# shaneson0/attacking_federate_learning

Measured on AMD Instinct MI355X. Metric: aggregation rounds/sec at N clients x D params (Bulyan), higher is better.
Workload: dtype f32 (Gram: fp16x2 split of every fp32 operand, 3 fp16 MFMAs per block, fp32/fp64 accumulate; <= 2e-7 of |gi||gj| vs f...

## Files before the change

### attacking_federate_learning_amd/csrc/gram_planes.hip

```cpp
#include "common.hpp"

#include <cstring>
#include <type_traits>

namespace byz {
namespace {

constexpr int kWgRows = 256;
constexpr int kWgCols = 128;
constexpr int kSlab = 128;
constexpr int kThreads = 512;
constexpr int kFragBytes = 1024;
constexpr int kRowBlocks = (kWgRows + kWgCols) / 32;
constexpr int kChunkCols = 8192;
constexpr int kChunkSteps = kChunkCols / 16;
constexpr int kFlushSteps = 16;
constexpr int kSpareRoundsPercent = 10;

typedef float f32x16 __attribute__((ext_vector_type(16)));
typedef float f32x4 __attribute__((ext_vector_type(4)));
typedef __bf16 bf16x8 __attribute__((ext_vector_type(8)));
typedef _Float16 f16x8 __attribute__((ext_vector_type(8)));
typedef uint32_t u32x4 __attribute__((ext_vector_type(4)));

__device__ __forceinline__ void split_bf16x3(const f32x4& lo4, const f32x4& hi4, u32x4& hp, u32x4& mp, u32x4& lp) {
    uint32_t xb[8], r1b[8], r2b[8];
#pragma unroll
    for (int e = 0; e < 8; ++e) {
        const float x = e < 4 ? lo4[e] : hi4[e - 4];
        xb[e] = __float_as_uint(x);
        const float r1 = x - __uint_as_float(xb[e] & 0xffff0000u);
        r1b[e] = __float_as_uint(r1);
        const float r2 = r1 - __uint_as_float(r1b[e] & 0xffff0000u);
        r2b[e] = __float_as_uint(r2);
    }
#pragma unroll
    for (int e = 0; e < 4; ++e) {
        hp[e] = __builtin_amdgcn_perm(xb[2 * e + 1], xb[2 * e], 0x07060302u);
        mp[e] = __builtin_amdgcn_perm(r1b[2 * e + 1], r1b[2 * e], 0x07060302u);
        lp[e] = __builtin_amdgcn_perm(r2b[2 * e + 1], r2b[2 * e], 0x07060302u);
    }
}

__device__ __forceinline__ void split_f16x2(const f32x4& lo4, const f32x4& hi4, float scale, u32x4& hp, u32x4& mp) {
    f16x8 h, m;
#pragma unroll
    for (int e = 0; e < 8; ++e) {
        const float x = (e < 4 ? lo4[e] : hi4[e - 4]) * scale;
        h[e] = static_cast<_Float16>(x);
        m[e] = static_cast<_Float16>(x - static_cast<float>(h[e]));
    }
    hp = __builtin_bit_cast(u32x4, h);
    mp = __builtin_bit_cast(u32x4, m);
}

__device__ __forceinline__ f32x4 load4_tail(const float* __restrict__ src, int64_t k, int64_t n_cols) {
    f32x4 v = {0.0f, 0.0f, 0.0f, 0.0f};
    if (k + 3 < n_cols) {
        v = *reinterpret_cast<const f32x4*>(src + k);
    } else {
        if (k + 0 < n_cols) v.x = src[k + 0];
        if (k + 1 < n_cols) v.y = src[k + 1];
        if (k + 2 < n_cols) v.z = src[k + 2];
    }
    return v;
}

constexpr int kSplitCols = 128;
__global__ __launch_bounds__(256) void plane_split_bf16_kernel(const float* __restrict__ G, int64_t n_rows, int64_t n_cols,
                                                               int64_t ld, const int32_t* __restrict__ row_index,
                                                               int64_t k0, int64_t n_steps, u32x4* __restrict__ planes) {
    __shared__ __attribute__((aligned(16))) float tile[32][kSplitCols + 4];
    const int tid = threadIdx.x;
    const int64_t rb = blockIdx.y;
    const int64_t step0 = static_cast<int64_t>(blockIdx.x) * (kSplitCols / 16);
    {
        const int r = tid >> 3, c = tid & 7;
        int64_t row = rb * 32 + r;
        if (row > n_rows - 1) row = n_rows - 1;
        if (row_index != nullptr) row = row_index[row];
        const float* src = G + row * ld;
#pragma unroll
        for (int p = 0; p < 4; ++p) {
            const int col = 4 * c + 32 * p;
            *reinterpret_cast<f32x4*>(&tile[r][col]) = load4_tail(src, k0 + step0 * 16 + col, n_cols);
        }
    }
    __syncthreads();
    const int lane = tid & 63, wave = tid >> 6;
#pragma unroll
    for (int i = 0; i < 2; ++i) {
        const int sl = 2 * wave + i;
        const int64_t step = step0 + sl;
        if (step >= n_steps) continue;
        const int row = lane & 31, kk = sl * 16 + 8 * (lane >> 5);
        const f32x4 lo4 = *reinterpret_cast<const f32x4*>(&tile[row][kk]);
        const f32x4 hi4 = *reinterpret_cast<const f32x4*>(&tile[row][kk + 4]);
        u32x4 h, m, l;
        split_bf16x3(lo4, hi4, h, m, l);
        u32x4* out = planes + ((rb * n_steps + step) * 3) * 64 + lane;
        out[0] = h;
        out[64] = m;
        out[128] = l;
    }
}

__global__ __launch_bounds__(256) void plane_split_f16_kernel(const float* __restrict__ G, int64_t n_rows, int64_t n_cols,
                                                              int64_t ld, const int32_t* __restrict__ row_index, int64_t k0,
                                                              int64_t n_steps, u32x4* __restrict__ planes,
                                                              double* __restrict__ unscale, int64_t rows_pad,
                                                              const int32_t* __restrict__ redo) {
    __shared__ __attribute__((aligned(16))) float tile[32][kSplitCols + 4];
    __shared__ float row_scale[32];
    const int tid = threadIdx.x;
    const int lane = tid & 63, wave = tid >> 6;
    const int listed = redo != nullptr ? redo[0] : 1;
    for (int item = redo != nullptr ? static_cast<int>(blockIdx.x) : 0; item < listed; item += static_cast<int>(gridDim.x)) {
    const int64_t rb = redo != nullptr ? redo[2 + 2 * item] : blockIdx.y;
    const int64_t chunk = redo != nullptr ? redo[1 + 2 * item] : blockIdx.x;
    const int r = tid >> 3, c = tid & 7;
    int64_t row = rb * 32 + r;
    if (row > n_rows - 1) row = n_rows - 1;
    if (row_index != nullptr) row = row_index[row];
    const float* src = G + row * ld;
    const int64_t kbeg = k0 + chunk * kChunkCols;
    {
        float mx = 0.0f;
        bool bad = false;
#pragma unroll 8
        for (int i = 0; i < kChunkCols / 32; ++i) {
            const f32x4 v = load4_tail(src, kbeg + 4 * c + 32 * i, n_cols);
#pragma unroll
            for (int e = 0; e < 4; ++e) {
                const float a = __builtin_fabsf(v[e]);
                bad = bad || !(a <= 3.0e38f);
                mx = __builtin_fmaxf(mx, a);
            }
        }
#pragma unroll
        for (int msk = 1; msk < 8; msk <<= 1) {
            mx = __builtin_fmaxf(mx, __shfl_xor(mx, msk, 64));
            bad = bad || (__shfl_xor(bad ? 1 : 0, msk, 64) != 0);
        }
        int shift = 0;
        if (!bad && mx > 0.0f) {
            shift = 14 - (static_cast<int>((__float_as_uint(mx) >> 23) & 0xffu) - 127);
            if (mx < 1.17549435e-38f) shift = 126;
            if (shift > 126) shift = 126;
            if (shift < -126) shift = -126;
        }
        if (c == 0) {
            row_scale[r] = __uint_as_float(static_cast<uint32_t>(shift + 127) << 23);
            unscale[chunk * rows_pad + rb * 32 + r] = __longlong_as_double(static_cast<long long>(1023 - shift) << 52);
        }
    }
    __syncthreads();
    const int64_t step_base = chunk * kChunkSteps;
    for (int sub = 0; sub < kChunkCols / kSplitCols; ++sub) {
        const int64_t step0 = step_base + sub * (kSplitCols / 16);
        if (step0 >= n_steps) break;
#pragma unroll
        for (int p = 0; p < 4; ++p) {
            const int col = 4 * c + 32 * p;
            *reinterpret_cast<f32x4*>(&tile[r][col]) = load4_tail(src, k0 + step0 * 16 + col, n_cols);
        }
        __syncthreads();
#pragma unroll
        for (int i = 0; i < 2; ++i) {
            const int sl = 2 * wave + i;
            const int64_t step = step0 + sl;
            if (step >= n_steps) continue;
            const int frow = lane & 31, kk = sl * 16 + 8 * (lane >> 5);
            const f32x4 lo4 = *reinterpret_cast<const f32x4*>(&tile[frow][kk]);
            const f32x4 hi4 = *reinterpret_cast<const f32x4*>(&tile[frow][kk + 4]);
            u32x4 h, m;
            split_f16x2(lo4, hi4, row_scale[frow], h, m);
            u32x4* out = planes + ((rb * n_steps + step) * 2) * 64 + lane;
            out[0] = h;
            out[64] = m;
        }
        __syncthreads();
    }
    if (redo == nullptr) break;
    __syncthreads();
    }
}

constexpr int kSampleGroups = 16;
__global__ __launch_bounds__(256) void plane_split_f16_stream_kernel(const float* __restrict__ G, int64_t n_rows, int64_t n_cols,
                                                                     int64_t ld, const int32_t* __restrict__ row_index, int64_t k0,
                                                                     int64_t n_steps, u32x4* __restrict__ planes,
                                                                     double* __restrict__ unscale, int64_t rows_pad,
                                                                     int32_t* __restrict__ redo) {
    __shared__ __attribute__((aligned(16))) float tile[2][32][kSplitCols + 4];
    __shared__ float row_scale[32];
    __shared__ int block_bad;
    const int tid = threadIdx.x;
    const int lane = tid & 63, wave = tid >> 6;
    const int64_t rb = blockIdx.y;
    const int64_t chunk = blockIdx.x;
    const int r = tid >> 3, c = tid & 7;
    int64_t row = rb * 32 + r;
    if (row > n_rows - 1) row = n_rows - 1;
    if (row_index != nullptr) row = row_index[row];
    const float* src = G + row * ld;
    const int64_t kbeg = k0 + chunk * kChunkCols;
    if (tid == 0) block_bad = 0;
    int shift = 0;
    {
        float mx = 0.0f;
#pragma unroll
        for (int g = 0; g < 2; ++g) {
            const int64_t k = kbeg + (2 * c + g) * (kChunkCols / kSampleGroups);
            const f32x4 a = load4_tail(src, k, n_cols), b = load4_tail(src, k + 4, n_cols);
#pragma unroll
            for (int e = 0; e < 4; ++e) mx = __builtin_fmaxf(mx, __builtin_fmaxf(__builtin_fabsf(a[e]), __builtin_fabsf(b[e])));
        }
#pragma unroll
        for (int msk = 1; msk < 8; msk <<= 1) mx = __builtin_fmaxf(mx, __shfl_xor(mx, msk, 64));
        if (mx >= 1.17549435e-38f && mx <= 3.0e38f) {
            shift = 9 - (static_cast<int>((__float_as_uint(mx) >> 23) & 0xffu) - 127);
            if (shift > 126) shift = 126;
            if (shift < -126) shift = -126;
        }
        if (c == 0) row_scale[r] = __uint_as_float(static_cast<uint32_t>(shift + 127) << 23);
    }
    const int64_t step_base = chunk * kChunkSteps;
    const float scale = __uint_as_float(static_cast<uint32_t>(shift + 127) << 23);
    float true_max = 0.0f;
    bool bad = false;
    f32x4 cur[4], nxt[4];
#pragma unroll
    for (int p = 0; p < 4; ++p) cur[p] = load4_tail(src, k0 + step_base * 16 + 4 * c + 32 * p, n_cols);
    __syncthreads();
    for (int sub = 0; sub < kChunkCols / kSplitCols; ++sub) {
        const int64_t step0 = step_base + sub * (kSplitCols / 16);
        if (step0 >= n_steps) break;
        const bool more = sub + 1 < kChunkCols / kSplitCols && step0 + kSplitCols / 16 < n_steps;
        if (more) {
#pragma unroll
            for (int p = 0; p < 4; ++p) nxt[p] = load4_tail(src, k0 + (step0 + kSplitCols / 16) * 16 + 4 * c + 32 * p, n_cols);
        }
        float (*t)[kSplitCols + 4] = tile[sub & 1];
#pragma unroll
        for (int p = 0; p < 4; ++p) {
            *reinterpret_cast<f32x4*>(&t[r][4 * c + 32 * p]) = cur[p];
#pragma unroll
            for (int e = 0; e < 4; ++e) {
                const float a = __builtin_fabsf(cur[p][e]);
                bad = bad || !(a <= 3.0e38f);
                true_max = __builtin_fmaxf(true_max, a);
            }
        }
        __syncthreads();
#pragma unroll
        for (int i = 0; i < 2; ++i) {
            const int sl = 2 * wave + i;
            const int64_t step = step0 + sl;
            if (step >= n_steps) continue;
            const int frow = lane & 31, kk = sl * 16 + 8 * (lane >> 5);
            const f32x4 lo4 = *reinterpret_cast<const f32x4*>(&t[frow][kk]);
            const f32x4 hi4 = *reinterpret_cast<const f32x4*>(&t[frow][kk + 4]);
            u32x4 h, m;
            split_f16x2(lo4, hi4, row_scale[frow], h, m);
            u32x4* out = planes + ((rb * n_steps + step) * 2) * 64 + lane;
            out[0] = h;
            out[64] = m;
        }
        if (more) {
#pragma unroll
            for (int p = 0; p < 4; ++p) cur[p] = nxt[p];
        }
    }
#pragma unroll
    for (int msk = 1; msk < 8; msk <<= 1) {
        true_max = __builtin_fmaxf(true_max, __shfl_xor(true_max, msk, 64));
        bad = bad || (__shfl_xor(bad ? 1 : 0, msk, 64) != 0);
    }
    const float scaled = true_max * scale;
    const bool holds = !bad && (true_max == 0.0f || (scaled >= 128.0f && scaled < 65536.0f));
    if (c == 0) {
        unscale[chunk * rows_pad + rb * 32 + r] = __longlong_as_double(static_cast<long long>(1023 - shift) << 52);
        if (!holds) block_bad = 1;
    }
    __syncthreads();
    if (tid == 0 && block_bad != 0) {
        const int at = atomicAdd(redo, 1);
        redo[1 + 2 * at] = static_cast<int32_t>(chunk);
        redo[2 + 2 * at] = static_cast<int32_t>(rb);
    }
}

template <int N>
__device__ __forceinline__ void wait_vmcnt() {
    asm volatile("s_waitcnt vmcnt(%0)" ::"n"(N) : "memory");
}
__device__ __forceinline__ void wait_vmcnt_dyn(int n) {
    switch (n) {
#define BYZ_W(k) case k: wait_vmcnt<k>(); break;
        BYZ_W(0) BYZ_W(3) BYZ_W(4) BYZ_W(5) BYZ_W(6) BYZ_W(8) BYZ_W(9) BYZ_W(10) BYZ_W(12) BYZ_W(15) BYZ_W(16) BYZ_W(18) BYZ_W(20) BYZ_W(24)
#undef BYZ_W
        default: wait_vmcnt<0>(); break;
    }
}

struct Frags {
    bf16x8 a[3][2], b[3][2];
};

template <int NBUF>
__global__ __launch_bounds__(512, 1) void gram_planes_kernel(const u32x4* __restrict__ planes, int64_t n_steps,
                                                             double* __restrict__ partial, int n_tiles,
                                                             const int2* __restrict__ tile_order, int n_chunks,
                                                             int* __restrict__ tickets, int round_size, int t128,
                                                             int slab_live0, int n_blocks32,
                                                             int32_t* __restrict__ device_status) {
    constexpr int PLANES = 3;
    constexpr int kRbBytes = PLANES * kFragBytes;
    constexpr int kStage = kRowBlocks * kRbBytes;
    constexpr int NW = 8;
    constexpr int kPieces = kRowBlocks * PLANES;
    constexpr int kPerWave = (kPieces + NW - 1) / NW;
    constexpr int kFullWaves = kPieces % NW == 0 ? NW : kPieces % NW;
    constexpr int kLead = NBUF;
    typedef bf16x8 frag_t;
    extern __shared__ __attribute__((aligned(16))) unsigned char lds[];

    const int xcd = blockIdx.x & 7;
    const int seq = blockIdx.x >> 3;
    const int base = n_tiles >> 3, rem = n_tiles & 7;
    const int mine = base + (xcd < rem ? 1 : 0);
    const int first = xcd * base + (xcd < rem ? xcd : rem);
    const int chunk = mine > 0 ? seq / mine : n_chunks;
    int* done = tickets + n_tiles + xcd;
    {
        const int round = round_size > 0 ? seq / round_size : 0;
        if (round > 0 && threadIdx.x == 0) {
            unsigned spins = 0;
            while (__hip_atomic_load(done, __ATOMIC_RELAXED, __HIP_MEMORY_SCOPE_AGENT) < round * round_size) {
                __builtin_amdgcn_s_sleep(16);
                if (++spins > (1u << 20)) break;
            }
        }
        __syncthreads();
        if (chunk >= n_chunks) {
            if (threadIdx.x == 0) __hip_atomic_fetch_add(done, 1, __ATOMIC_RELAXED, __HIP_MEMORY_SCOPE_AGENT);
            return;
        }
    }
    const int t_list = first + (seq - chunk * mine);
    const int2 tt = tile_order[t_list];
    const int bi = __builtin_amdgcn_readfirstlane(tt.x);
    const int tj = __builtin_amdgcn_readfirstlane(tt.y);

    const int tid = threadIdx.x;
    const int lane = tid & 63;
    const int wave = __builtin_amdgcn_readfirstlane(tid >> 6);
    const int wr = wave >> 1, wc = wave & 1;
    const int ti = 2 * bi + wr / 2;
    const int row_in_slab = (wr % 2) * 64;
    unsigned live_blocks = 0;
    if (tj <= ti && ti < t128 && n_blocks32 < 0) {
        live_blocks = 15u;
    } else if (tj <= ti && ti < t128) {
#pragma unroll
        for (int m = 0; m < 2; ++m)
#pragma unroll
            for (int n = 0; n < 2; ++n) {
                const int rblk = ti * 4 + row_in_slab / 32 + m, cblk = tj * 4 + wc * 2 + n;
                if (rblk < n_blocks32 && cblk <= rblk) live_blocks |= 1u << (m * 2 + n);
            }
    }
    const bool live_wave = live_blocks != 0;

    const int step0 = chunk * kChunkSteps;
    int n_stages = static_cast<int>(n_steps) - step0;
    if (n_stages > kChunkSteps) n_stages = kChunkSteps;

    int64_t piece_off[kPerWave];
#pragma unroll
    for (int i = 0; i < kPerWave; ++i) {
        int q = wave + NW * i;
        if (q >= kPieces) q = kPieces - 1;
        const int rbl = q / PLANES, piece = q % PLANES;
        const int64_t rb = rbl < 8 ? static_cast<int64_t>(bi) * 8 + rbl : static_cast<int64_t>(tj) * 4 + (rbl - 8);
        piece_off[i] = (((rb * n_steps + step0) * PLANES + piece) * 64) * 16;
    }
    const unsigned char* lane_base = reinterpret_cast<const unsigned char*>(planes) + lane * 16;
    const int my_dmas = wave < kFullWaves ? kPerWave : kPerWave - 1;
    auto dma = [&](int s) __attribute__((always_inline)) {
        unsigned char* dst = lds + (s % NBUF) * kStage + wave * kFragBytes;
#pragma unroll
        for (int i = 0; i < kPerWave; ++i) {
            if (kFullWaves != NW && i == kPerWave - 1 && wave >= kFullWaves) break;
            __builtin_amdgcn_global_load_lds(
                (const __attribute__((address_space(1))) void*)(lane_base + piece_off[i] + static_cast<int64_t>(s) * (PLANES * kFragBytes)),
                (__attribute__((address_space(3))) void*)(dst + i * NW * kFragBytes), 16, 0, 0);
        }
    };

    f32x16 acc[2][2], acc2[2][2];
#pragma unroll
    for (int m = 0; m < 2; ++m)
#pragma unroll
        for (int n = 0; n < 2; ++n)
#pragma unroll
            for (int e = 0; e < 16; ++e) {
                acc[m][n][e] = 0.0f;
                acc2[m][n][e] = 0.0f;
            }

    auto read_frags = [&](int s, Frags& f, auto mask_c) __attribute__((always_inline)) {
        constexpr unsigned MASK = decltype(mask_c)::value;
        const unsigned char* A = lds + (s % NBUF) * kStage + (2 * wr) * kRbBytes + lane * 16;
        const unsigned char* B = lds + (s % NBUF) * kStage + (8 + 2 * wc) * kRbBytes + lane * 16;
#pragma unroll
        for (int p = 0; p < PLANES; ++p) {
#pragma unroll
            for (int m = 0; m < 2; ++m)
                if (((MASK >> (m * 2)) & 3u) != 0) f.a[p][m] = *reinterpret_cast<const frag_t*>(A + m * kRbBytes + p * kFragBytes);
#pragma unroll
            for (int n = 0; n < 2; ++n)
                if (((MASK >> n) & 5u) != 0) f.b[p][n] = *reinterpret_cast<const frag_t*>(B + n * kRbBytes + p * kFragBytes);
        }
    };
    auto multiply = [&](const Frags& f, auto mask_c) __attribute__((always_inline)) {
        constexpr unsigned MASK = decltype(mask_c)::value;
        constexpr int pa[6] = {2, 0, 1, 1, 0, 0};
        constexpr int pb[6] = {0, 2, 1, 0, 1, 0};
#pragma unroll
        for (int t = 0; t < 6; ++t)
#pragma unroll
            for (int m = 0; m < 2; ++m)
#pragma unroll
                for (int n = 0; n < 2; ++n)
                    if (((MASK >> (m * 2 + n)) & 1u) != 0)
                        acc[m][n] = __builtin_amdgcn_mfma_f32_32x32x16_bf16(f.a[pa[t]][m], f.b[pb[t]][n], acc[m][n], 0, 0, 0);
    };
    auto flush = [&](int s) __attribute__((always_inline)) {
        if ((s + 1) % kFlushSteps == 0) {
#pragma unroll
            for (int m = 0; m < 2; ++m)
#pragma unroll
                for (int n = 0; n < 2; ++n)
#pragma unroll
                    for (int e = 0; e < 16; ++e) {
                        acc2[m][n][e] += acc[m][n][e];
                        acc[m][n][e] = 0.0f;
                    }
        }
    };
    auto steady = [&](int s, const Frags& cur, Frags& next, auto mask_c) __attribute__((always_inline)) {
        constexpr bool kLive = decltype(mask_c)::value != 0;
        dma(s + kLead);
        if (kLive) {
            read_frags(s + 1, next, mask_c);
            multiply(cur, mask_c);
        }
        if (kFullWaves == NW || wave < kFullWaves) wait_vmcnt<(kLead - 2) * kPerWave>();
        else wait_vmcnt<(kLead - 2) * (kPerWave - 1)>();
        asm volatile("s_waitcnt lgkmcnt(0)\n\ts_barrier" ::: "memory");
        if (kLive) flush(s);
    };
    auto drain = [&](int s, const Frags& cur, Frags& next, auto mask_c) __attribute__((always_inline)) {
        constexpr bool kLive = decltype(mask_c)::value != 0;
        if (s + kLead < n_stages) dma(s + kLead);
        if (kLive) {
            if (s + 1 < n_stages) read_frags(s + 1, next, mask_c);
            multiply(cur, mask_c);
        }
        const int last = s + kLead < n_stages ? s + kLead : n_stages - 1;
        const int ahead = last - (s + 2);
        wait_vmcnt_dyn((ahead > 0 ? ahead : 0) * my_dmas);
        asm volatile("s_waitcnt lgkmcnt(0)\n\ts_barrier" ::: "memory");
        if (kLive) flush(s);
    };

    for (int a = 0; a < kLead && a < n_stages; ++a) dma(a);
    {
        const int issued = n_stages < kLead ? n_stages : kLead;
        wait_vmcnt_dyn((issued > 2 ? issued - 2 : 0) * my_dmas);
    }
    asm volatile("s_barrier" ::: "memory");
    auto k_loop = [&](auto mask_c) __attribute__((always_inline)) {
        constexpr bool kLive = decltype(mask_c)::value != 0;
        Frags x, y;
        if (kLive && n_stages > 0) read_frags(0, x, mask_c);
        asm volatile("s_waitcnt lgkmcnt(0)\n\ts_barrier" ::: "memory");
        int s = 0;
        for (; s + 1 + kLead < n_stages; s += 2) {
            steady(s, x, y, mask_c);
            steady(s + 1, y, x, mask_c);
        }
        for (; s < n_stages; s += 2) {
            drain(s, x, y, mask_c);
            if (s + 1 < n_stages) drain(s + 1, y, x, mask_c);
        }
    };
    switch (live_blocks) {
        case 0u: k_loop(std::integral_constant<unsigned, 0u>{}); break;
        case 1u: k_loop(std::integral_constant<unsigned, 1u>{}); break;
        case 3u: k_loop(std::integral_constant<unsigned, 3u>{}); break;
        case 13u: k_loop(std::integral_constant<unsigned, 13u>{}); break;
        default: live_blocks = 15u; k_loop(std::integral_constant<unsigned, 15u>{}); break;
    }
    auto block_live = [&](int m, int n) __attribute__((always_inline)) { return ((live_blocks >> (m * 2 + n)) & 1u) != 0; };

    bool lost = false;
    if (chunk > 0) {
        if (tid == 0) {
            unsigned spins = 0;
            while (__hip_atomic_load(tickets + t_list, __ATOMIC_RELAXED, __HIP_MEMORY_SCOPE_AGENT) != chunk) {
                __builtin_amdgcn_s_sleep(8);
                if (++spins > (1u << 26)) {
                    lost = true;
                    break;
                }
            }
            __builtin_amdgcn_fence(__ATOMIC_ACQUIRE, "agent");
        }
        lost = __syncthreads_or(lost ? 1 : 0) != 0;
    }
    if (lost) {
        if (tid == 0) atomicOr(device_status, kStatusLostTicket);
    } else if (live_wave) {
        const bool slab_live = chunk > 0 || slab_live0 != 0;
        double* out = partial + (static_cast<int64_t>(ti) * (ti + 1) / 2 + tj) * (kSlab * kSlab);
#pragma unroll
        for (int m = 0; m < 2; ++m)
#pragma unroll
            for (int n = 0; n < 2; ++n) {
                if (!block_live(m, n)) continue;
                const int j = wc * 64 + n * 32 + (lane & 31);
#pragma unroll
                for (int e = 0; e < 16; ++e) {
                    const int i = row_in_slab + m * 32 + (e & 3) + 8 * (e >> 2) + 4 * (lane >> 5);
                    double v = static_cast<double>(acc2[m][n][e]);
                    v += static_cast<double>(acc[m][n][e]);
                    if (slab_live) v += out[i * kSlab + j];
                    out[i * kSlab + j] = v;
                }
            }
    }
    asm volatile("s_waitcnt vmcnt(0)" ::: "memory");
    __syncthreads();
    if (tid == 0) {
        __builtin_amdgcn_fence(__ATOMIC_RELEASE, "agent");
        asm volatile("s_waitcnt vmcnt(0)" ::: "memory");
        __hip_atomic_store(tickets + t_list, chunk + 1, __ATOMIC_RELAXED, __HIP_MEMORY_SCOPE_AGENT);
        __hip_atomic_fetch_add(done, 1, __ATOMIC_RELAXED, __HIP_MEMORY_SCOPE_AGENT);
    }
}

template <int NBUF, bool DEFER>
__global__ __launch_bounds__(512, 1) void gram_planes16_kernel(const u32x4* __restrict__ planes, int64_t n_steps,
                                                            const double* __restrict__ unscale, int64_t rows_pad,
                                                            double* __restrict__ partial, int n_tiles,
                                                            const int2* __restrict__ tile_order, int n_chunks,
                                                            int* __restrict__ tickets, int round_size, int run, int t128,
                                                            int slab_live0, int n_blocks32,
                                                            int32_t* __restrict__ device_status,
                                                            float* __restrict__ chunk_sums,
                                                            float* __restrict__ ragged_sums) {
    constexpr int PLANES = 2;
    constexpr int kRbBytes = PLANES * kFragBytes;
    constexpr int kStage = kRowBlocks * kRbBytes;
    constexpr int NW = 8;
    constexpr int kPerWave = kRowBlocks * PLANES / NW;
    constexpr int kSuperFlush = kFlushSteps / 2;
    static_assert(kRowBlocks * PLANES % NW == 0 && NBUF == 6, "ring arithmetic below");
    typedef f16x8 frag_t;
    extern __shared__ __attribute__((aligned(16))) unsigned char lds[];

    const int xcd = blockIdx.x & 7;
    const int seq = blockIdx.x >> 3;
    int* done = tickets + n_tiles + xcd;
    __shared__ int claimed_round;
    {
        const int round = round_size > 0 ? seq / round_size : 0;
        if (round > 0 && threadIdx.x == 0) {
            unsigned spins = 0;
            while (__hip_atomic_load(done, __ATOMIC_RELAXED, __HIP_MEMORY_SCOPE_AGENT) < round * round_size) {
                __builtin_amdgcn_s_sleep(16);
                if (++spins > (1u << 20)) break;
            }
        }
        if (threadIdx.x == 0) {
            int* slot = tickets + n_tiles + 9 + xcd * static_cast<int>(gridDim.x / (8u * static_cast<unsigned>(run))) + seq / run;
            int v = __hip_atomic_load(slot, __ATOMIC_RELAXED, __HIP_MEMORY_SCOPE_AGENT);
            if (v == 0) {
                int expected = 0;
                if (__hip_atomic_compare_exchange_strong(slot, &expected, -1, __ATOMIC_RELAXED, __ATOMIC_RELAXED, __HIP_MEMORY_SCOPE_AGENT)) {
                    v = __hip_atomic_fetch_add(tickets + n_tiles + 8, 1, __ATOMIC_RELAXED, __HIP_MEMORY_SCOPE_AGENT) + 1;
                    __hip_atomic_store(slot, v, __ATOMIC_RELAXED, __HIP_MEMORY_SCOPE_AGENT);
                } else {
                    v = expected;
                }
            }
            while (v <= 0) {
                __builtin_amdgcn_s_sleep(1);
                v = __hip_atomic_load(slot, __ATOMIC_RELAXED, __HIP_MEMORY_SCOPE_AGENT);
            }
            claimed_round = v - 1;
        }
        __syncthreads();
    }
    const int unit = __builtin_amdgcn_readfirstlane(claimed_round * run + seq % run);
    const int chunk = __builtin_amdgcn_readfirstlane(unit / n_tiles);
    if (chunk >= n_chunks) {
        if (threadIdx.x == 0) __hip_atomic_fetch_add(done, 1, __ATOMIC_RELAXED, __HIP_MEMORY_SCOPE_AGENT);
        return;
    }
    const int t_list = unit - chunk * n_tiles;
    const int2 tt = tile_order[t_list];
    const int bi = __builtin_amdgcn_readfirstlane(tt.x);
    const int tj = __builtin_amdgcn_readfirstlane(tt.y);

    const int tid = threadIdx.x;
    const int lane = tid & 63;
    const int wave = __builtin_amdgcn_readfirstlane(tid >> 6);
    const int wr = wave >> 1, wc = wave & 1;
    const int ti = 2 * bi + wr / 2;
    const int row_in_slab = (wr % 2) * 64;
    unsigned live_blocks = 0;
    if (tj <= ti && ti < t128 && n_blocks32 < 0) {
        live_blocks = 15u;
    } else if (tj <= ti && ti < t128) {
#pragma unroll
        for (int m = 0; m < 2; ++m)
#pragma unroll
            for (int n = 0; n < 2; ++n) {
                const int rblk = ti * 4 + row_in_slab / 32 + m, cblk = tj * 4 + wc * 2 + n;
                if (rblk < n_blocks32 && cblk <= rblk) live_blocks |= 1u << (m * 2 + n);
            }
    }
    const bool live_wave = live_blocks != 0;

    const int step0 = chunk * kChunkSteps;
    int n_stages = static_cast<int>(n_steps) - step0;
    if (n_stages > kChunkSteps) n_stages = kChunkSteps;
    const int n_super = n_stages / 2;

    int64_t piece_off[kPerWave];
#pragma unroll
    for (int i = 0; i < kPerWave; ++i) {
        const int q = wave + NW * i;
        const int rbl = q / PLANES, piece = q % PLANES;
        const int64_t rb = rbl < 8 ? static_cast<int64_t>(bi) * 8 + rbl : static_cast<int64_t>(tj) * 4 + (rbl - 8);
        piece_off[i] = (((rb * n_steps + step0) * PLANES + piece) * 64) * 16;
    }
    const unsigned char* lane_base = reinterpret_cast<const unsigned char*>(planes) + lane * 16;
    auto dma_piece = [&](int s, int i) __attribute__((always_inline)) {
        unsigned char* dst = lds + (s % NBUF) * kStage + wave * kFragBytes;
        __builtin_amdgcn_global_load_lds(
            (const __attribute__((address_space(1))) void*)(lane_base + piece_off[i] + static_cast<int64_t>(s) * (PLANES * kFragBytes)),
            (__attribute__((address_space(3))) void*)(dst + i * NW * kFragBytes), 16, 0, 0);
    };
    auto dma = [&](int s) __attribute__((always_inline)) {
#pragma unroll
        for (int i = 0; i < kPerWave; ++i) dma_piece(s, i);
    };

    f32x4 acc[4][4], acc2[4][4];
#pragma unroll
    for (int m = 0; m < 4; ++m)
#pragma unroll
        for (int n = 0; n < 4; ++n)
#pragma unroll
            for (int e = 0; e < 4; ++e) {
                acc[m][n][e] = 0.0f;
                acc2[m][n][e] = 0.0f;
            }

    const int lane_in_image = (lane & 15) + 32 * ((lane >> 4) & 1);
    const int pair_half = lane >> 5;
    auto frag_at = [&](int sp, int rb32, int h, int p) __attribute__((always_inline)) -> frag_t {
        const unsigned char* at = lds + (2 * (sp % (NBUF / 2)) + pair_half) * kStage + rb32 * kRbBytes + p * kFragBytes +
                                  (lane_in_image + 16 * h) * 16;
        return *reinterpret_cast<const frag_t*>(at);
    };
    struct AFrags { frag_t v[2][4]; };
    struct BFrags { frag_t v[2][2]; };
    auto read_a = [&](int sp, AFrags& a, auto mask_c) __attribute__((always_inline)) {
        constexpr unsigned MASK = decltype(mask_c)::value;
#pragma unroll
        for (int p = 0; p < 2; ++p)
#pragma unroll
            for (int m = 0; m < 4; ++m)
                if (((MASK >> ((m / 2) * 2)) & 3u) != 0) a.v[p][m] = frag_at(sp, 2 * wr + m / 2, m % 2, p);
    };
    auto read_b = [&](int sp, int half, BFrags& b, auto mask_c) __attribute__((always_inline)) {
        constexpr unsigned MASK = decltype(mask_c)::value;
#pragma unroll
        for (int p = 0; p < 2; ++p)
#pragma unroll
            for (int n = 0; n < 2; ++n) b.v[p][n] = frag_at(sp, 8 + 2 * wc + half, n, p);
        (void)MASK;
    };
    auto multiply_half = [&](const AFrags& a, const BFrags& b, auto half_c, auto mask_c) __attribute__((always_inline)) {
        constexpr unsigned MASK = decltype(mask_c)::value;
        constexpr int HALF = decltype(half_c)::value;
        constexpr int pa[3] = {1, 0, 0};
        constexpr int pb[3] = {0, 1, 0};
#pragma unroll
        for (int t = 0; t < 3; ++t)
#pragma unroll
            for (int m = 0; m < 4; ++m)
#pragma unroll
                for (int n = 0; n < 2; ++n)
                    if (((MASK >> ((m / 2) * 2 + HALF)) & 1u) != 0)
                        acc[m][2 * HALF + n] = __builtin_amdgcn_mfma_f32_16x16x32_f16(a.v[pa[t]][m], b.v[pb[t]][n], acc[m][2 * HALF + n], 0, 0, 0);
    };
    auto flush = [&](int sp) __attribute__((always_inline)) {
        if ((sp + 1) % kSuperFlush == 0) {
#pragma unroll
            for (int m = 0; m < 4; ++m)
#pragma unroll
                for (int n = 0; n < 4; ++n)
#pragma unroll
                    for (int e = 0; e < 4; ++e) {
                        acc2[m][n][e] += acc[m][n][e];
                        acc[m][n][e] = 0.0f;
                    }
        }
    };

    for (int a = 0; a < NBUF && a < n_stages; ++a) dma(a);
    {
        const int issued = n_stages < NBUF ? n_stages : NBUF;
        wait_vmcnt_dyn((issued > 2 ? issued - 2 : 0) * kPerWave);
    }
    asm volatile("s_barrier" ::: "memory");
    auto k_loop = [&](auto mask_c) __attribute__((always_inline)) {
        constexpr unsigned MASK = decltype(mask_c)::value;
        constexpr bool kLive = MASK != 0;
        constexpr std::integral_constant<int, 0> h0{};
        constexpr std::integral_constant<int, 1> h1{};
        AFrags a0, a1;
        BFrags b0, b1;
        if (kLive && n_super > 0) {
            read_a(0, a0, mask_c);
            if ((MASK & 5u) != 0) read_b(0, 0, b0, mask_c);
        }
        auto super = [&](int sp, AFrags& a, AFrags& an) __attribute__((always_inline)) {
            if (kLive) {
                if ((MASK & 10u) != 0) read_b(sp, 1, b1, mask_c);
                if ((MASK & 5u) != 0) multiply_half(a, b0, h0, mask_c);
            }
            {
                const int last = 2 * sp + 5 < n_stages - 1 ? 2 * sp + 5 : n_stages - 1;
                const int ahead = last - (2 * sp + 3);
                if (2 * sp + 7 < n_stages) wait_vmcnt<2 * kPerWave>();
                else wait_vmcnt_dyn((ahead > 0 ? ahead : 0) * kPerWave);
            }
            asm volatile("s_waitcnt lgkmcnt(0)\n\ts_barrier" ::: "memory");
            if (2 * sp + NBUF < n_stages) dma(2 * sp + NBUF);
            if (2 * sp + NBUF + 1 < n_stages) dma(2 * sp + NBUF + 1);
            if (kLive) {
                if (sp + 1 < n_super) {
                    read_a(sp + 1, an, mask_c);
                    if ((MASK & 5u) != 0) read_b(sp + 1, 0, b0, mask_c);
                }
                if ((MASK & 10u) != 0) multiply_half(a, b1, h1, mask_c);
                flush(sp);
            }
        };
        auto super8 = [&](int sp, AFrags& a, AFrags& an, auto pos_c) __attribute__((always_inline)) {
            constexpr int POS = decltype(pos_c)::value;
            constexpr bool FRESH = POS == 0, FLUSHING = POS == 7;
            constexpr int pa[3] = {1, 0, 0};
            constexpr int pb[3] = {0, 1, 0};
            const f32x4 zero4 = {0.0f, 0.0f, 0.0f, 0.0f};
#pragma unroll
            for (int g = 0; g < 4; ++g) {
                b1.v[g / 2][g % 2] = frag_at(sp, 8 + 2 * wc + 1, g % 2, g / 2);
#pragma unroll
                for (int q = 6 * g; q < 6 * g + 6; ++q) {
                    const int t = q / 8, m = (q % 8) / 2, n = q % 2;
                    acc[m][n] = __builtin_amdgcn_mfma_f32_16x16x32_f16(a.v[pa[t]][m], b0.v[pb[t]][n], (FRESH && t == 0) ? zero4 : acc[m][n], 0, 0, 0);
                }
                __builtin_amdgcn_sched_barrier(0);
            }
            wait_vmcnt<2 * kPerWave>();
            asm volatile("s_waitcnt lgkmcnt(0)\n\ts_barrier" ::: "memory");
#pragma unroll
            for (int g = 0; g < 6; ++g) {
                dma_piece(2 * sp + NBUF + g / 3, g % 3);
#pragma unroll
                for (int r = 2 * g; r < 2 * g + 2; ++r) {
                    if (r < 8) an.v[r / 4][r % 4] = frag_at(sp + 1, 2 * wr + (r % 4) / 2, (r % 4) % 2, r / 4);
                    else b0.v[(r - 8) / 2][(r - 8) % 2] = frag_at(sp + 1, 8 + 2 * wc + 0, (r - 8) % 2, (r - 8) / 2);
                }
#pragma unroll
                for (int q = 4 * g; q < 4 * g + 4; ++q) {
                    const int t = q / 8, m = (q % 8) / 2, n = q % 2;
                    acc[m][2 + n] = __builtin_amdgcn_mfma_f32_16x16x32_f16(a.v[pa[t]][m], b1.v[pb[t]][n], (FRESH && t == 0) ? zero4 : acc[m][2 + n], 0, 0, 0);
                }
                if constexpr (FLUSHING) {
#pragma unroll
                    for (int b = (8 * g) / 6; b < (8 * (g + 1)) / 6; ++b)
#pragma unroll
                        for (int e = 0; e < 4; ++e) acc2[b / 2][b % 2][e] += acc[b / 2][b % 2][e];
                }
                __builtin_amdgcn_sched_barrier(0);
            }
            if constexpr (FLUSHING) {
#pragma unroll
                for (int m = 0; m < 4; ++m)
#pragma unroll
                    for (int n = 2; n < 4; ++n)
#pragma unroll
                        for (int e = 0; e < 4; ++e) acc2[m][n][e] += acc[m][n][e];
            }
        };
        int sp = 0;
        if constexpr (MASK == 15u) {
            bool any = false;
            for (; 2 * (sp + 7) + NBUF + 1 < n_stages && sp + 8 < n_super; sp += 8) {
                super8(sp + 0, a0, a1, std::integral_constant<int, 0>{});
                super8(sp + 1, a1, a0, std::integral_constant<int, 1>{});
                super8(sp + 2, a0, a1, std::integral_constant<int, 2>{});
                super8(sp + 3, a1, a0, std::integral_constant<int, 3>{});
                super8(sp + 4, a0, a1, std::integral_constant<int, 4>{});
                super8(sp + 5, a1, a0, std::integral_constant<int, 5>{});
                super8(sp + 6, a0, a1, std::integral_constant<int, 6>{});
                super8(sp + 7, a1, a0, std::integral_constant<int, 7>{});
                any = true;
            }
            if (any) {
#pragma unroll
                for (int m = 0; m < 4; ++m)
#pragma unroll
                    for (int n = 0; n < 4; ++n)
#pragma unroll
                        for (int e = 0; e < 4; ++e) acc[m][n][e] = 0.0f;
            }
        }
        for (; sp + 1 < n_super; sp += 2) {
            super(sp, a0, a1);
            super(sp + 1, a1, a0);
        }
        if (sp < n_super) super(sp, a0, a1);
    };
    switch (live_blocks) {
        case 0u: k_loop(std::integral_constant<unsigned, 0u>{}); break;
        case 1u: k_loop(std::integral_constant<unsigned, 1u>{}); break;
        case 3u: k_loop(std::integral_constant<unsigned, 3u>{}); break;
        case 13u: k_loop(std::integral_constant<unsigned, 13u>{}); break;
        default: live_blocks = 15u; k_loop(std::integral_constant<unsigned, 15u>{}); break;
    }
    auto block_live = [&](int m, int n) __attribute__((always_inline)) { return ((live_blocks >> ((m / 2) * 2 + n / 2)) & 1u) != 0; };

    if constexpr (DEFER) {
        if (live_wave) {
            const int sel = wr / 2;
            const bool unflushed = (n_super % kSuperFlush) != 0;
            float* out = chunk_sums + ((static_cast<int64_t>(chunk) * n_tiles + t_list) * 2 + sel) * (kSlab * kSlab);
            float* rag = ragged_sums + (static_cast<int64_t>(t_list) * 2 + sel) * (kSlab * kSlab);
#pragma unroll
            for (int m = 0; m < 4; ++m)
#pragma unroll
                for (int n = 0; n < 4; ++n) {
                    if (!block_live(m, n)) continue;
                    const int j = wc * 64 + 16 * n + (lane & 15);
#pragma unroll
                    for (int e = 0; e < 4; ++e) {
                        const int i = row_in_slab + 16 * m + 4 * (lane >> 4) + e;
                        out[i * kSlab + j] = acc2[m][n][e];
                        if (unflushed) rag[i * kSlab + j] = acc[m][n][e];
                    }
                }
        }
        __syncthreads();
        if (tid == 0) __hip_atomic_fetch_add(done, 1, __ATOMIC_RELAXED, __HIP_MEMORY_SCOPE_AGENT);
        return;
    }
    bool lost = false;
    if (chunk > 0) {
        if (tid == 0) {
            unsigned spins = 0;
            while (__hip_atomic_load(tickets + t_list, __ATOMIC_RELAXED, __HIP_MEMORY_SCOPE_AGENT) != chunk) {
                __builtin_amdgcn_s_sleep(8);
                if (++spins > (1u << 26)) {
                    lost = true;
                    break;
                }
            }
            __builtin_amdgcn_fence(__ATOMIC_ACQUIRE, "agent");
        }
        lost = __syncthreads_or(lost ? 1 : 0) != 0;
    }
    if (lost) {
        if (tid == 0) atomicOr(device_status, kStatusLostTicket);
    } else if (live_wave) {
        const bool slab_live = chunk > 0 || slab_live0 != 0;
        double* out = partial + (static_cast<int64_t>(ti) * (ti + 1) / 2 + tj) * (kSlab * kSlab);
        const double* un = unscale + static_cast<int64_t>(chunk) * rows_pad;
#pragma unroll
        for (int m = 0; m < 4; ++m)
#pragma unroll
            for (int n = 0; n < 4; ++n) {
                if (!block_live(m, n)) continue;
                const int j = wc * 64 + 16 * n + (lane & 15);
                const double uj = un[static_cast<int64_t>(tj) * kSlab + j];
#pragma unroll
                for (int e = 0; e < 4; ++e) {
                    const int i = row_in_slab + 16 * m + 4 * (lane >> 4) + e;
                    double v = static_cast<double>(acc2[m][n][e]);
                    v += static_cast<double>(acc[m][n][e]);
                    v *= un[static_cast<int64_t>(ti) * kSlab + i] * uj;
                    if (slab_live) v += out[i * kSlab + j];
                    out[i * kSlab + j] = v;
                }
            }
    }
    asm volatile("s_waitcnt vmcnt(0)" ::: "memory");
    __syncthreads();
    if (tid == 0) {
        __builtin_amdgcn_fence(__ATOMIC_RELEASE, "agent");
        asm volatile("s_waitcnt vmcnt(0)" ::: "memory");
        __hip_atomic_store(tickets + t_list, chunk + 1, __ATOMIC_RELAXED, __HIP_MEMORY_SCOPE_AGENT);
        __hip_atomic_fetch_add(done, 1, __ATOMIC_RELAXED, __HIP_MEMORY_SCOPE_AGENT);
    }
}

constexpr int kReduceRun = 8;
__global__ __launch_bounds__(256) void chunk_reduce_kernel(const float* __restrict__ chunk_sums, const float* __restrict__ ragged_sums,
                                                           int n_tiles, int n_chunks, int ragged_chunk,
                                                           const int2* __restrict__ tile_order, const double* __restrict__ unscale,
                                                           int64_t rows_pad, double* __restrict__ partial, int slab_live0,
                                                           int t128, int n_blocks32) {
    typedef double f64x4 __attribute__((ext_vector_type(4)));
    const int t_list = blockIdx.x >> 1, sel = blockIdx.x & 1;
    const int2 tt = tile_order[t_list];
    const int ti = 2 * tt.x + sel, tj = tt.y;
    if (!(tj <= ti && ti < t128)) return;
    double* out = partial + (static_cast<int64_t>(ti) * (ti + 1) / 2 + tj) * (kSlab * kSlab);
    const int64_t slab_stride = static_cast<int64_t>(n_tiles) * 2 * (kSlab * kSlab);
    const float* in = chunk_sums + (static_cast<int64_t>(t_list) * 2 + sel) * (kSlab * kSlab);
    const float* rag = ragged_sums + (static_cast<int64_t>(t_list) * 2 + sel) * (kSlab * kSlab);
    const int i = static_cast<int>(blockIdx.y) * 32 + (threadIdx.x >> 3), j = (threadIdx.x & 7) * 4;
    for (int jb = 0; jb < kSlab; jb += 32) {
        const int jj = jb + j;
        if (n_blocks32 >= 0) {
            const int rblk = ti * 4 + (i >> 5), cblk = tj * 4 + (jj >> 5);
            if (!(rblk < n_blocks32 && cblk <= rblk)) continue;
        }
        const int idx = i * kSlab + jj;
        f64x4 v = {0.0, 0.0, 0.0, 0.0};
        bool live = slab_live0 != 0;
        if (live) v = *reinterpret_cast<const f64x4*>(out + idx);
        for (int c0 = 0; c0 < n_chunks; c0 += kReduceRun) {
            f32x4 p[kReduceRun];
            double ui[kReduceRun];
            f64x4 uj[kReduceRun];
#pragma unroll
            for (int k = 0; k < kReduceRun; ++k) {
                const int c = c0 + k < n_chunks ? c0 + k : n_chunks - 1;
                p[k] = *reinterpret_cast<const f32x4*>(in + c * slab_stride + idx);
                const double* un = unscale + static_cast<int64_t>(c) * rows_pad;
                ui[k] = un[static_cast<int64_t>(ti) * kSlab + i];
                uj[k] = *reinterpret_cast<const f64x4*>(un + static_cast<int64_t>(tj) * kSlab + jj);
            }
#pragma unroll
            for (int k = 0; k < kReduceRun; ++k) {
                if (c0 + k >= n_chunks) break;
                f64x4 q = {static_cast<double>(p[k][0]), static_cast<double>(p[k][1]), static_cast<double>(p[k][2]),
                           static_cast<double>(p[k][3])};
                if (c0 + k == ragged_chunk) {
                    const f32x4 r = *reinterpret_cast<const f32x4*>(rag + idx);
                    q[0] += static_cast<double>(r[0]); q[1] += static_cast<double>(r[1]);
                    q[2] += static_cast<double>(r[2]); q[3] += static_cast<double>(r[3]);
                }
#pragma unroll
                for (int e = 0; e < 4; ++e) {
                    q[e] *= ui[k] * uj[k][e];
                    v[e] = live ? q[e] + v[e] : q[e];
                }
                live = true;
            }
        }
        *reinterpret_cast<f64x4*>(out + idx) = v;
    }
}

}

bool gram_planes_enabled() { return env_int("BYZ_GRAM_PLANES", 1) != 0; }

int launch_gram_planes(byz_ctx* ctx, const float* G, int64_t n_rows, int64_t n_cols, int64_t ld, const int32_t* row_index,
                       double* slabs, int share_count, int share_index, uint8_t* owned_host, bool f16, hipStream_t stream) {
    const int64_t t128 = ceil_div(n_rows, kSlab);
    const int64_t t256 = ceil_div(t128, 2);
    const int64_t rows_pad = t256 * kWgRows;
    const int64_t order_key = static_cast<int64_t>(f16 ? 1 : 0) * (1ll << 40) + share_count * 65536 + share_index;
    if (ctx->plane_order_T != t128 || ctx->plane_order_share != order_key) {
        ctx->plane_order_host.clear();
        int64_t position = 0;
        auto push = [&](int64_t bi, int64_t tj) {
            if (position++ % share_count != share_index) return;
            ctx->plane_order_host.push_back(static_cast<int32_t>(bi));
            ctx->plane_order_host.push_back(static_cast<int32_t>(tj));
        };
        if (f16) {
            for (int64_t b0 = 0; b0 < t256; b0 += 4)
                for (int64_t tj = 0; tj < t128 && tj <= 2 * (b0 + 3) + 1; ++tj)
                    for (int64_t bi = b0; bi < b0 + 4 && bi < t256; ++bi)
                        if (tj <= 2 * bi + 1) push(bi, tj);
        } else {
            const int64_t S = ceil_div(t128, 8);
            for (int64_t I = 0; I < S; ++I)
                for (int64_t J = 0; J <= I; ++J)
                    for (int64_t bi = I * 4; bi < I * 4 + 4 && bi < t256; ++bi)
                        for (int64_t tj = J * 8; tj < J * 8 + 8 && tj <= 2 * bi + 1 && tj < t128; ++tj) push(bi, tj);
        }
        BYZ_TRY(ctx->plane_order.ensure(ctx->plane_order_host.size() * sizeof(int32_t) + 16));
        BYZ_HIP(hipMemcpyAsync(ctx->plane_order.ptr, ctx->plane_order_host.data(),
                               ctx->plane_order_host.size() * sizeof(int32_t), hipMemcpyHostToDevice, stream));
        BYZ_HIP(hipStreamSynchronize(stream));
        ctx->plane_order_T = t128;
        ctx->plane_order_share = order_key;
    }
    const int64_t n_tiles = static_cast<int64_t>(ctx->plane_order_host.size() / 2);
    if (owned_host != nullptr)
        for (int64_t t = 0; t < n_tiles; ++t) {
            const int64_t bi = ctx->plane_order_host[2 * t], tj = ctx->plane_order_host[2 * t + 1];
            for (int64_t ti = 2 * bi; ti < 2 * bi + 2 && ti < t128; ++ti)
                if (tj <= ti) owned_host[ti * (ti + 1) / 2 + tj] = 1;
        }
    if (n_tiles == 0) return BYZ_OK;

    const int n_planes = f16 ? 2 : 3;
    size_t free_b = 0, total_b = 0;
    BYZ_HIP(hipMemGetInfo(&free_b, &total_b));
    int64_t budget = static_cast<int64_t>(env_int("BYZ_GRAM_PLANE_MB", 16384)) << 20;
    const int64_t have = static_cast<int64_t>(ctx->gram_planes.bytes);
    if (budget > have + static_cast<int64_t>(free_b / 2)) budget = have + static_cast<int64_t>(free_b / 2);
    int64_t chunks_per_sc = budget / (rows_pad * 2 * n_planes * kChunkCols);
    const int64_t chunks_total = ceil_div(n_cols, kChunkCols);
    if (chunks_per_sc > chunks_total) chunks_per_sc = chunks_total;
    if (chunks_per_sc < 1) {
        set_error("gram: no room for one 8192-column chunk of 16-bit planes (%lld rows)", (long long)rows_pad);
        return BYZ_E_HIP;
    }
    const int64_t n_sc = ceil_div(chunks_total, chunks_per_sc);
    chunks_per_sc = ceil_div(chunks_total, n_sc);
    const int64_t sc_cols = chunks_per_sc * kChunkCols;
    BYZ_TRY(ctx->gram_planes.ensure(static_cast<size_t>(rows_pad) * 2 * n_planes * sc_cols));
    double* unscale = nullptr;
    if (f16) {
        BYZ_TRY(ctx->plane_unscale.ensure(static_cast<size_t>(rows_pad) * chunks_per_sc * sizeof(double)));
        unscale = ctx->plane_unscale.as<double>();
    }
    u32x4* planes = ctx->gram_planes.as<u32x4>();
    bool defer = f16 && env_int("BYZ_GRAM_DEFER", 1) != 0;
    float* chunk_sums = nullptr;
    float* ragged_sums = nullptr;
    if (defer) {
        const size_t per_chunk = static_cast<size_t>(n_tiles) * 2 * kSlab * kSlab * sizeof(float);
        const size_t want = per_chunk * static_cast<size_t>(chunks_per_sc + 1);
        size_t free_now = 0, total_now = 0;
        BYZ_HIP(hipMemGetInfo(&free_now, &total_now));
        if (want > ctx->gram_chunk_sums.bytes && want - ctx->gram_chunk_sums.bytes > free_now / 2) defer = false;
    }
    if (defer) {
        const size_t per_chunk = static_cast<size_t>(n_tiles) * 2 * kSlab * kSlab * sizeof(float);
        BYZ_TRY(ctx->gram_chunk_sums.ensure(per_chunk * static_cast<size_t>(chunks_per_sc + 1)));
        chunk_sums = ctx->gram_chunk_sums.as<float>();
        ragged_sums = chunk_sums + (per_chunk / sizeof(float)) * static_cast<size_t>(chunks_per_sc);
    }
    auto kernel16 = defer ? &gram_planes16_kernel<6, true> : &gram_planes16_kernel<6, false>;
    const void* kernel = f16 ? reinterpret_cast<const void*>(kernel16) : reinterpret_cast<const void*>(&gram_planes_kernel<4>);
    const size_t lds_bytes = static_cast<size_t>(f16 ? 6 : 4) * kRowBlocks * n_planes * kFragBytes;
    BYZ_HIP(allow_dynamic_lds(ctx, kernel, static_cast<int>(lds_bytes)));
    const int round_size = env_int("BYZ_GRAM_ROUND", ctx->num_cus / 8);
    const int run = round_size > 0 ? round_size : ctx->num_cus / 8;
    const int n_blocks32 = env_int("BYZ_GRAM_BLOCK_SKIP", 1) != 0 ? static_cast<int>(ceil_div(n_rows, 32)) : -1;
    const int64_t per_xcd = ceil_div(n_tiles, 8);
    for (int64_t sc = 0; sc < n_sc; ++sc) {
        const int64_t k0 = sc * sc_cols;
        const int64_t cols = n_cols - k0 < sc_cols ? n_cols - k0 : sc_cols;
        const int64_t n_steps = ceil_div(cols, 32) * 2;
        const int64_t n_chunks = ceil_div(n_steps, kChunkSteps);
        {
            KernelTimer t(ctx, BYZ_K_PLANE_SPLIT, stream);
            if (f16) {
                const dim3 grid(static_cast<unsigned>(n_chunks), static_cast<unsigned>(rows_pad / 32));
                if (env_int("BYZ_GRAM_SPLIT_TWO_PASS", 0) != 0) {
                    plane_split_f16_kernel<<<grid, 256, 0, stream>>>(G, n_rows, n_cols, ld, row_index, k0, n_steps, planes,
                                                                     unscale, rows_pad, nullptr);
                } else {
                    const int64_t pairs = n_chunks * (rows_pad / 32);
                    BYZ_TRY(ctx->split_redo.ensure(static_cast<size_t>(1 + 2 * pairs) * sizeof(int32_t)));
                    int32_t* redo = ctx->split_redo.as<int32_t>();
                    BYZ_HIP(hipMemsetAsync(redo, 0, sizeof(int32_t), stream));
                    plane_split_f16_stream_kernel<<<grid, 256, 0, stream>>>(G, n_rows, n_cols, ld, row_index, k0, n_steps, planes,
                                                                            unscale, rows_pad, redo);
                    BYZ_TRY(check_launch("plane_split_f16_stream_kernel"));
                    const int64_t fix = pairs < 4096 ? pairs : 4096;
                    plane_split_f16_kernel<<<static_cast<unsigned>(fix), 256, 0, stream>>>(G, n_rows, n_cols, ld, row_index, k0,
                                                                                           n_steps, planes, unscale, rows_pad, redo);
                }
            } else {
                const dim3 grid(static_cast<unsigned>(ceil_div(n_steps, kSplitCols / 16)), static_cast<unsigned>(rows_pad / 32));
                plane_split_bf16_kernel<<<grid, 256, 0, stream>>>(G, n_rows, n_cols, ld, row_index, k0, n_steps, planes);
            }
            BYZ_TRY(check_launch("plane_split_kernel"));
        }
        {
            int64_t rounds_per_xcd = 0;
            if (f16) {
                rounds_per_xcd = ceil_div(ceil_div(n_tiles * n_chunks, run), 8);
                rounds_per_xcd += rounds_per_xcd * kSpareRoundsPercent / 100;
            }
            const int64_t grid = f16 ? 8 * run * rounds_per_xcd : 8 * per_xcd * n_chunks;
            const size_t ticket_ints = static_cast<size_t>(n_tiles + 9 + 8 * rounds_per_xcd);
            BYZ_TRY(ctx->gram_tickets.ensure(ticket_ints * sizeof(int)));
            int* tickets = ctx->gram_tickets.as<int>();
            BYZ_HIP(hipMemsetAsync(tickets, 0, ticket_ints * sizeof(int), stream));
            KernelTimer t(ctx, BYZ_K_GRAM, stream);
            if (grid > 0x7fffffff) {
                set_error("gram: grid too large");
                return BYZ_E_UNSUPPORTED;
            }
            const int2* tile_order = ctx->plane_order.as<int2>();
            const int slab_live0 = sc > 0 ? 1 : 0;
            if (!f16) {
                gram_planes_kernel<4><<<static_cast<unsigned>(grid), kThreads, lds_bytes, stream>>>(
                    planes, n_steps, slabs, static_cast<int>(n_tiles), tile_order, static_cast<int>(n_chunks), tickets,
                    round_size, static_cast<int>(t128), slab_live0, n_blocks32, device_status_word(ctx));
            } else {
                kernel16<<<static_cast<unsigned>(grid), kThreads, lds_bytes, stream>>>(
                    planes, n_steps, unscale, rows_pad, slabs, static_cast<int>(n_tiles), tile_order, static_cast<int>(n_chunks),
                    tickets, round_size, run, static_cast<int>(t128), slab_live0, n_blocks32, device_status_word(ctx),
                    chunk_sums, ragged_sums);
            }
            BYZ_TRY(check_launch("gram_planes_kernel"));
        }
        if (defer) {
            KernelTimer t(ctx, BYZ_K_GRAM_REDUCE, stream);
            const int ragged_chunk = (n_steps % kChunkSteps) % kFlushSteps != 0 ? static_cast<int>(n_chunks) - 1 : -1;
            chunk_reduce_kernel<<<dim3(static_cast<unsigned>(2 * n_tiles), 4), 256, 0, stream>>>(
                chunk_sums, ragged_sums, static_cast<int>(n_tiles), static_cast<int>(n_chunks), ragged_chunk,
                ctx->plane_order.as<int2>(), unscale, rows_pad, slabs, sc > 0 ? 1 : 0, static_cast<int>(t128), n_blocks32);
            BYZ_TRY(check_launch("chunk_reduce_kernel"));
        }
    }
    return BYZ_OK;
}

}
```

Baseline: 2.055.

## Redistribute live 16x16 blocks evenly across waves for ragged and diagonal tiles

For tiles where only part of the rows are valid (ragged edge) or on the diagonal, the work of live 16-row blocks is re-dealt across waves with explicit row/column selections, so no wave sits idle while others do all the MFMAs. A new templated k-loop handles K dealt blocks per wave with per-block LDS offsets, and the epilogues are generalised to map dealt rows and columns back to output positions. This aims to cut the critical path of load-imbalanced workgroups, at the cost of more code paths, extra register state and more complex index mapping.

After: 2.045. Within noise of the previous version (-0.5%).

```diff
diff --git a/attacking_federate_learning_amd/csrc/gram_planes.hip b/attacking_federate_learning_amd/csrc/gram_planes.hip
--- a/attacking_federate_learning_amd/csrc/gram_planes.hip
+++ b/attacking_federate_learning_amd/csrc/gram_planes.hip
@@ -634,7 +634,40 @@
                 if (rblk < n_blocks32 && cblk <= rblk) live_blocks |= 1u << (m * 2 + n);
             }
     }
-    const bool live_wave = live_blocks != 0;
+    int deal = 0;
+    int row_sel[4] = {0, 0, 0, 0};
+    int col_sel[2] = {0, 0};
+    if (n_blocks32 >= 0) {
+        const int valid = n_blocks32 - 8 * bi;
+        const bool diagonal = tj >= 2 * bi;
+        if (valid < 8 && !diagonal) {
+            deal = valid;
+            const int q = wave & 3, c0 = 2 * (wave >> 2);
+            if (valid <= 4) {
+                col_sel[0] = c0 + (q >> 1);
+#pragma unroll
+                for (int m = 0; m < 4; ++m) row_sel[m] = (q & 1) * valid + (m < valid ? m : 0);
+            } else {
+                const int e = valid - 4, base = (q >> 1) * (4 + e);
+                col_sel[0] = c0 + (q & 1);
+                col_sel[1] = c0 + 1 - (q & 1);
+#pragma unroll
+                for (int m = 0; m < 4; ++m) row_sel[m] = (q & 1) == 0 ? base + m : base + e + 3 - m;
+            }
+        } else if (valid >= 8 && diagonal) {
+            if (wave < 4) {
+                deal = 5;
+                const unsigned rows = wave == 0 ? 0x3102u : wave == 1 ? 0x7654u : wave == 2 ? 0x7536u : 0x6547u;
+                const int shift = tj == 2 * bi ? 0 : 8;
+#pragma unroll
+                for (int m = 0; m < 4; ++m) row_sel[m] = static_cast<int>((rows >> (4 * m)) & 15u) + shift;
+                col_sel[0] = wave < 2 ? 0 : wave - 1;
+                col_sel[1] = wave < 2 ? 1 : 3;
+            } else if (tj != 2 * bi) {
+                live_blocks = 0;
+            }
+        }
+    }
 
     const int step0 = chunk * kChunkSteps;
     int n_stages = static_cast<int>(n_steps) - step0;
@@ -731,6 +764,90 @@
         wait_vmcnt_dyn((issued > 2 ? issued - 2 : 0) * kPerWave);
     }
     asm volatile("s_barrier" ::: "memory");
+    int a_off[4], b_off[2];
+#pragma unroll
+    for (int m = 0; m < 4; ++m) a_off[m] = (row_sel[m] >> 1) * kRbBytes + (row_sel[m] & 1) * 256;
+#pragma unroll
+    for (int h = 0; h < 2; ++h) b_off[h] = (8 + col_sel[h]) * kRbBytes;
+    auto frag_off = [&](int sp, int off, int p) __attribute__((always_inline)) -> frag_t {
+        const unsigned char* at = lds + (2 * (sp % (NBUF / 2)) + pair_half) * kStage + off + p * kFragBytes + lane_in_image * 16;
+        return *reinterpret_cast<const frag_t*>(at);
+    };
+    auto k_loop_dealt = [&](auto k_c) __attribute__((always_inline)) {
+        constexpr int K = decltype(k_c)::value;
+        constexpr int NA = K < 4 ? K : 4;
+        constexpr int NB = K > 4 ? K - 4 : 0;
+        constexpr int pa[3] = {1, 0, 0};
+        constexpr int pb[3] = {0, 1, 0};
+        AFrags a0, a1;
+        BFrags b0, b1;
+        auto read_a = [&](int sp, AFrags& a) __attribute__((always_inline)) {
+#pragma unroll
+            for (int p = 0; p < 2; ++p)
+#pragma unroll
+                for (int m = 0; m < NA; ++m) a.v[p][m] = frag_off(sp, a_off[m], p);
+        };
+        auto read_b = [&](int sp, int half, BFrags& b) __attribute__((always_inline)) {
+#pragma unroll
+            for (int p = 0; p < 2; ++p)
+#pragma unroll
+                for (int n = 0; n < 2; ++n) b.v[p][n] = frag_off(sp, b_off[half] + n * 256, p);
+        };
+        auto multiply = [&](const AFrags& a, const BFrags& b, auto half_c) __attribute__((always_inline)) {
+            constexpr int HALF = decltype(half_c)::value;
+            constexpr int ROWS = HALF == 0 ? NA : NB;
+#pragma unroll
+            for (int t = 0; t < 3; ++t)
+#pragma unroll
+                for (int m = 0; m < ROWS; ++m)
+#pragma unroll
+                    for (int n = 0; n < 2; ++n)
+                        acc[m][2 * HALF + n] = __builtin_amdgcn_mfma_f32_16x16x32_f16(a.v[pa[t]][m], b.v[pb[t]][n], acc[m][2 * HALF + n], 0, 0, 0);
+        };
+        constexpr std::integral_constant<int, 0> h0{};
+        constexpr std::integral_constant<int, 1> h1{};
+        if (n_super > 0) {
+            read_a(0, a0);
+            read_b(0, 0, b0);
+        }
+        auto super = [&](int sp, AFrags& a, AFrags& an) __attribute__((always_inline)) {
+            if (NB > 0) read_b(sp, 1, b1);
+            multiply(a, b0, h0);
+            {
+                const int last = 2 * sp + 5 < n_stages - 1 ? 2 * sp + 5 : n_stages - 1;
+                const int ahead = last - (2 * sp + 3);
+                if (2 * sp + 7 < n_stages) wait_vmcnt<2 * kPerWave>();
+                else wait_vmcnt_dyn((ahead > 0 ? ahead : 0) * kPerWave);
+            }
+            asm volatile("s_waitcnt lgkmcnt(0)\n\ts_barrier" ::: "memory");
+            if (2 * sp + NBUF < n_stages) dma(2 * sp + NBUF);
+            if (2 * sp + NBUF + 1 < n_stages) dma(2 * sp + NBUF + 1);
+            if (sp + 1 < n_super) {
+                read_a(sp + 1, an);
+                read_b(sp + 1, 0, b0);
+            }
+            if (NB > 0) multiply(a, b1, h1);
+            if ((sp + 1) % kSuperFlush == 0) {
+#pragma unroll
+                for (int m = 0; m < NA; ++m)
+#pragma unroll
+                    for (int n = 0; n < 4; ++n)
+                        if (n < 2 || m < NB) {
+#pragma unroll
+                            for (int e = 0; e < 4; ++e) {
+                                acc2[m][n][e] += acc[m][n][e];
+                                acc[m][n][e] = 0.0f;
+                            }
+                        }
+            }
+        };
+        int sp = 0;
+        for (; sp + 1 < n_super; sp += 2) {
+            super(sp, a0, a1);
+            super(sp + 1, a1, a0);
+        }
+        if (sp < n_super) super(sp, a0, a1);
+    };
     auto k_loop = [&](auto mask_c) __attribute__((always_inline)) {
         constexpr unsigned MASK = decltype(mask_c)::value;
         constexpr bool kLive = MASK != 0;
@@ -842,34 +959,56 @@
         }
         if (sp < n_super) super(sp, a0, a1);
     };
-    switch (live_blocks) {
-        case 0u: k_loop(std::integral_constant<unsigned, 0u>{}); break;
-        case 1u: k_loop(std::integral_constant<unsigned, 1u>{}); break;
-        case 3u: k_loop(std::integral_constant<unsigned, 3u>{}); break;
-        case 13u: k_loop(std::integral_constant<unsigned, 13u>{}); break;
-        default: live_blocks = 15u; k_loop(std::integral_constant<unsigned, 15u>{}); break;
-    }
-    auto block_live = [&](int m, int n) __attribute__((always_inline)) { return ((live_blocks >> ((m / 2) * 2 + n / 2)) & 1u) != 0; };
+    if (deal != 0) {
+        switch (deal) {
+            case 1: k_loop_dealt(std::integral_constant<int, 1>{}); break;
+            case 2: k_loop_dealt(std::integral_constant<int, 2>{}); break;
+            case 3: k_loop_dealt(std::integral_constant<int, 3>{}); break;
+            case 4: k_loop_dealt(std::integral_constant<int, 4>{}); break;
+            case 5: k_loop_dealt(std::integral_constant<int, 5>{}); break;
+            case 6: k_loop_dealt(std::integral_constant<int, 6>{}); break;
+            default: k_loop_dealt(std::integral_constant<int, 7>{}); break;
+        }
+    } else {
+        switch (live_blocks) {
+            case 0u: k_loop(std::integral_constant<unsigned, 0u>{}); break;
+            case 1u: k_loop(std::integral_constant<unsigned, 1u>{}); break;
+            case 3u: k_loop(std::integral_constant<unsigned, 3u>{}); break;
+            case 13u: k_loop(std::integral_constant<unsigned, 13u>{}); break;
+            default: live_blocks = 15u; k_loop(std::integral_constant<unsigned, 15u>{}); break;
+        }
+    }
+    int row16[4];
+#pragma unroll
+    for (int m = 0; m < 4; ++m) row16[m] = deal != 0 ? row_sel[m] : 4 * wr + m;
+    auto col16 = [&](int n) __attribute__((always_inline)) { return deal != 0 ? 2 * col_sel[n / 2] + n % 2 : 4 * wc + n; };
+    auto block_live = [&](int m, int n) __attribute__((always_inline)) {
+        if (deal != 0) return m + 4 * (n / 2) < deal;
+        return ((live_blocks >> ((m / 2) * 2 + n / 2)) & 1u) != 0;
+    };
+    const bool live_wave = deal != 0 || live_blocks != 0;
 
     if constexpr (DEFER) {
         if (live_wave) {
-            const int sel = wr / 2;
             const bool unflushed = (n_super % kSuperFlush) != 0;
-            float* out = chunk_sums + ((static_cast<int64_t>(chunk) * n_tiles + t_list) * 2 + sel) * (kSlab * kSlab);
-            float* rag = ragged_sums + (static_cast<int64_t>(t_list) * 2 + sel) * (kSlab * kSlab);
-#pragma unroll
-            for (int m = 0; m < 4; ++m)
+#pragma unroll
+            for (int m = 0; m < 4; ++m) {
+                const int sel = row16[m] >> 3;
+                const int i0 = (row16[m] & 7) * 16;
+                float* out = chunk_sums + ((static_cast<int64_t>(chunk) * n_tiles + t_list) * 2 + sel) * (kSlab * kSlab);
+                float* rag = ragged_sums + (static_cast<int64_t>(t_list) * 2 + sel) * (kSlab * kSlab);
 #pragma unroll
                 for (int n = 0; n < 4; ++n) {
                     if (!block_live(m, n)) continue;
-                    const int j = wc * 64 + 16 * n + (lane & 15);
+                    const int j = 16 * col16(n) + (lane & 15);
 #pragma unroll
                     for (int e = 0; e < 4; ++e) {
-                        const int i = row_in_slab + 16 * m + 4 * (lane >> 4) + e;
+                        const int i = i0 + 4 * (lane >> 4) + e;
                         out[i * kSlab + j] = acc2[m][n][e];
                         if (unflushed) rag[i * kSlab + j] = acc[m][n][e];
                     }
                 }
+            }
         }
         __syncthreads();
         if (tid == 0) __hip_atomic_fetch_add(done, 1, __ATOMIC_RELAXED, __HIP_MEMORY_SCOPE_AGENT);
@@ -894,25 +1033,28 @@
         if (tid == 0) atomicOr(device_status, kStatusLostTicket);
     } else if (live_wave) {
         const bool slab_live = chunk > 0 || slab_live0 != 0;
-        double* out = partial + (static_cast<int64_t>(ti) * (ti + 1) / 2 + tj) * (kSlab * kSlab);
         const double* un = unscale + static_cast<int64_t>(chunk) * rows_pad;
 #pragma unroll
-        for (int m = 0; m < 4; ++m)
+        for (int m = 0; m < 4; ++m) {
+            const int64_t si = 2 * bi + (row16[m] >> 3);
+            const int i0 = (row16[m] & 7) * 16;
+            double* out = partial + (si * (si + 1) / 2 + tj) * (kSlab * kSlab);
 #pragma unroll
             for (int n = 0; n < 4; ++n) {
                 if (!block_live(m, n)) continue;
-                const int j = wc * 64 + 16 * n + (lane & 15);
+                const int j = 16 * col16(n) + (lane & 15);
                 const double uj = un[static_cast<int64_t>(tj) * kSlab + j];
 #pragma unroll
                 for (int e = 0; e < 4; ++e) {
-                    const int i = row_in_slab + 16 * m + 4 * (lane >> 4) + e;
+                    const int i = i0 + 4 * (lane >> 4) + e;
                     double v = static_cast<double>(acc2[m][n][e]);
                     v += static_cast<double>(acc[m][n][e]);
-                    v *= un[static_cast<int64_t>(ti) * kSlab + i] * uj;
+                    v *= un[si * kSlab + i] * uj;
                     if (slab_live) v += out[i * kSlab + j];
                     out[i * kSlab + j] = v;
                 }
             }
+        }
     }
     asm volatile("s_waitcnt vmcnt(0)" ::: "memory");
     __syncthreads();
```
